# atoms-ufrj/atomsmm

Hardware: AMD Instinct MI355X
Metric: ns/day on 100k-atom TIP3P RESPA box; near-nonbonded HBM GB/s vs 8 TB/s peak (higher is better)
Workload: dtype f64

## Files before the change

### atomsmm_amd/csrc/cluster.h

```cpp
#pragma once
#include "amm_ctx.h"

struct ClusterList {
    int nc = 0;
    const int *d_first = nullptr;
    const int *d_rest = nullptr;
    int nrest = 0;
    bool built = false;
    CellGrid grid;
    int capc = 0;
    int parts = 1;
    int *d_slice_cells = nullptr;
    int split_parts = 0;
    double rext = 0;
    double rlist_build = 0, rnear_build = 0, skin = 0;
    int *d_cell_count = nullptr, *d_cell_start = nullptr, *d_cell_members = nullptr;
    int *d_cperm = nullptr;
    int *d_aperm = nullptr;
    float4 *d_pos4f = nullptr;
    double *d_xref = nullptr;
    int c_begin = 0, c_end = 0;
    int cap = 0;
    int lpa = 8;
    int *d_nl = nullptr, *d_nnb = nullptr, *d_nnb_near = nullptr;
    int *d_flags = nullptr;
    unsigned long long *d_counters = nullptr;
    unsigned long long *d_blockstats = nullptr;
    int *d_ticket = nullptr;
    long checked_epoch = -1, pre_epoch = -1;
    const double *checked_pos = nullptr, *pre_pos = nullptr;
    PairForce *sorted_for = nullptr;
    long sorted_epoch = -1;
    const double *sorted_pos = nullptr;
    int *d_spec_count[2] = {nullptr, nullptr};
    int *d_spec_ticket = nullptr;
    int spec_parity = 0;
    long assigned_epoch = -1;
    const double *assigned_pos = nullptr;
    double built_L[3] = {0, 0, 0};
// ... 14 lines not shown
```

### atomsmm_amd/csrc/cluster.hip

```cpp
#include <algorithm>
#include <cmath>
#include <cstdio>
#include <cstdlib>
#include <cstring>
#include <type_traits>
#include <vector>

#include "amm_ctx.h"
#include "bonded_terms.h"
#include "cluster.h"
#include "device_utils.h"
#include "pair_math.h"
#include "pair_tab.h"

#ifndef AMM_EXP_NOLJ
#define AMM_EXP_NOLJ 0
#endif

__device__ double amm_erfcx_table_dev_c[AMM_ERFCX_NI * AMM_ERFCX_NC];
static bool g_erfcx_uploaded_c[64] = {false};

void amm_cluster_classify(int n, const std::vector<int> &ptr, const std::vector<int> &idx, std::vector<int> &mol_first, std::vector<int> &rest) {
    mol_first.clear();
    rest.clear();
// ... 69 lines not shown

__device__ __forceinline__ double csorted_image(double x, double x0, double sh, double L, double invL) {
    return x + (sh - L * rint((x - x0) * invL));
}

__device__ __forceinline__ void cgather_one(int c, int i0, const double *__restrict__ pos, Box box, const double *__restrict__ q,
                                            const double *__restrict__ hsig, const double *__restrict__ seps2, double4 *posq_s, double2 *lj_s) {
    double sh[3];
#pragma unroll
    for (int k = 0; k < 3; ++k) sh[k] = cwrap1(pos[3 * i0 + k], box.L[k], box.invL[k]) - pos[3 * i0 + k];
#pragma unroll
    for (int a = 0; a < 3; ++a) {
        const int i = i0 + a;
        double4 p;
        p.x = csorted_image(pos[3 * i], pos[3 * i0], sh[0], box.L[0], box.invL[0]);
        p.y = csorted_image(pos[3 * i + 1], pos[3 * i0 + 1], sh[1], box.L[1], box.invL[1]);
        p.z = csorted_image(pos[3 * i + 2], pos[3 * i0 + 2], sh[2], box.L[2], box.invL[2]);
        p.w = q[i];
        posq_s[3 * c + a] = p;
        lj_s[3 * c + a] = make_double2(hsig[i], seps2[i]);
    }
}

__global__ void __launch_bounds__(256) k_csort_gather(int ncell, int nc, const int *__restrict__ start, const int *__restrict__ members,
                                                      int capc, int *cperm, int *aperm, const double *__restrict__ pos, Box box,
                                                      float4 *pos4f, const int *flags, int *wflags, int force, const double *__restrict__ q,
                                                      const double *__restrict__ hsig, const double *__restrict__ seps2, double4 *posq_s,
                                                      double2 *lj_s, float rext, const double *__restrict__ site_eps,
                                                      const int *__restrict__ first, CZeroRows Z, int copies_current, double *xref,
                                                      int c_begin, int c_end, int *slice_cells) {
    const int gid = blockIdx.x * blockDim.x + threadIdx.x;
    if (gid < Z.n) {
        const int i = Z.idx[gid];
        if (Z.f0) Z.f0[3 * i] = Z.f0[3 * i + 1] = Z.f0[3 * i + 2] = 0.0;
        if (Z.f1) Z.f1[3 * i] = Z.f1[3 * i + 1] = Z.f1[3 * i + 2] = 0.0;
    }
    if (!force && !flags[0]) {
        if (!copies_current && posq_s && gid < nc) cgather_one(gid, cfirst(first, cperm[gid]), pos, box, q, hsig, seps2, posq_s, lj_s);
        return;
    }
    const int wave = gid >> 6, lane = threadIdx.x & 63;
    if (wave >= ncell) return;
    const int b = start[wave];
    const int cnt = min(start[wave + 1] - b, capc);
    if (lane == 0 && c_begin < c_end) {
        if (b <= c_begin && c_begin < start[wave + 1]) slice_cells[0] = wave;
        if (b <= c_end - 1 && c_end - 1 < start[wave + 1]) slice_cells[1] = wave;
    }
    const int *mem = members + (size_t)wave * capc;
    for (int a0 = 0; a0 < cnt; a0 += 64) {
        const int a = a0 + lane;
        const int me = a < cnt ? mem[a] : 0x7fffffff;
        int rank = 0;
// ... 25 lines not shown
            const double z = csorted_image(pos[3 * i + 2], p0[2], sh[2], box.L[2], box.invL[2]);
            if (xref) {
                xref[3 * i] = pos[3 * i];
                xref[3 * i + 1] = pos[3 * i + 1];
                xref[3 * i + 2] = pos[3 * i + 2];
            }
            pf[t] = make_float4((float)x, (float)y, (float)z, 0.f);
            const float dx = pf[t].x - pf[0].x, dy = pf[t].y - pf[0].y, dz = pf[t].z - pf[0].z;
            ext2 = fmaxf(ext2, dx * dx + dy * dy + dz * dz);
            if (site_eps[i] != 0.0) sites |= 1 << t;
            if (posq_s) {
                posq_s[3 * sl + t] = make_double4(x, y, z, q[i]);
                lj_s[3 * sl + t] = make_double2(hsig[i], seps2[i]);
            }
        }
        const float ext = sqrtf(ext2) * 1.000001f + 1e-6f;
        if (!(ext <= rext)) wflags[7] = 1;
        pf[0].w = ext;
        pf[1].w = __int_as_float(sites);
        pos4f[3 * sl] = pf[0];
        pos4f[3 * sl + 1] = pf[1];
        pos4f[3 * sl + 2] = pf[2];
    }
}

struct CBoxF {
    float L[3], invL[3];
};

#ifndef CB_BATCH
#define CB_BATCH 5
#endif
#define CB_COARSE 256
#define CB_QCAP 256
__device__ __forceinline__ int cq_wrap(int i) { return i & (CB_QCAP - 1); }
typedef float v2f __attribute__((ext_vector_type(2)));

__device__ void cfinish_build_block(int *flags, unsigned long long *counters, const unsigned long long *blockstats, int nblocks, int count_only) {
    __shared__ unsigned long long sh_part[4][3];
    unsigned long long sum = 0, mx = 0, nr = 0;
    for (int b0 = threadIdx.x; b0 < nblocks; b0 += 8 * 256) {
        unsigned long long v[8][3];
#pragma unroll
        for (int j = 0; j < 8; ++j) {
            const int b = b0 + j * 256;
            const bool in = b < nblocks;
#pragma unroll
            for (int q = 0; q < 3; ++q) v[j][q] = in ? amm_ld_l2(&blockstats[3 * (in ? b : 0) + q]) : 0ull;
        }
#pragma unroll
        for (int j = 0; j < 8; ++j) {
            sum += v[j][0];
            mx = max(mx, v[j][1]);
            nr += v[j][2];
        }
    }
// ... 14 lines not shown
        counters[2] = sh_part[0][2] + sh_part[1][2] + sh_part[2][2] + sh_part[3][2];
        if (!count_only) {
            flags[0] = 0;
            flags[AMM_FLAG_FAR] = 0;
            counters[0] += 1;
        }
    }
}

#ifndef CB_WAVES
#define CB_WAVES 5
#endif
#define CB_OCC __attribute__((amdgpu_waves_per_eu(CB_WAVES)))
#ifdef AMM_CBS_TIMING
__device__ unsigned long long g_cbs_t[8];
#define CBS_STAMP(i) do { const unsigned long long now_ = wall_clock64(); if (w == 0 && lane == 0) atomicAdd(&g_cbs_t[i], now_ - t_last); t_last = now_; } while (0)
#else
#define CBS_STAMP(i) do { } while (0)
#endif
template <bool COUNT_ONLY, bool RINT, bool SLICE = false>
__global__ void __launch_bounds__(256) __attribute__((amdgpu_waves_per_eu(SLICE ? 3 : CB_WAVES))) k_cbuild(int c_begin, int c_end, int parts, const int *__restrict__ cell_start,
                                                const float4 *__restrict__ pos4f, CBoxF box, CellGrid g, float rlist, float rnear2, int cap,
                                                int *nl, int *nnb, int *nnb_near, int *flags, unsigned long long *blockstats,
                                                unsigned long long *counters, int *ticket, int force, const int *slice_cells) {
    if (!force && !flags[0]) return;
    __shared__ int s_rstart[4][128];
    __shared__ int s_rpref[4][128];
    __shared__ float s_rshift[4][3][128];
    __shared__ int s_q[4][CB_BATCH][CB_QCAP];
    __shared__ unsigned char s_coarse[4][CB_COARSE];
    const int lane = threadIdx.x & 63, w = threadIdx.x >> 6;
    const int wave = __builtin_amdgcn_readfirstlane((int)((blockIdx.x * blockDim.x + threadIdx.x) >> 6));
    const float FAR = 1.0e9f;
    const float rlist2 = rlist * rlist;
    unsigned long long wsum = 0, wnear = 0;
    int wmax = 0;
    const int first_cell = SLICE ? __builtin_amdgcn_readfirstlane(slice_cells[0]) : 0;
    const int nunits = SLICE ? (__builtin_amdgcn_readfirstlane(slice_cells[1]) - first_cell + 1) * parts : g.ncell * parts;
    int unit = wave;
#ifdef AMM_CBS_TIMING
    unsigned long long t_last = wall_clock64(), t_drain = 0, n_drain = 0;
#endif
    do {
    const int c = unit < nunits ? first_cell + unit / parts : g.ncell, part = unit % parts;
    int a_begin = 0, a_end = 0;
    if (c < g.ncell) {
        const int cb0 = __builtin_amdgcn_readfirstlane(cell_start[c]), cb1 = __builtin_amdgcn_readfirstlane(cell_start[c + 1]);
        const int per = (cb1 - cb0 + parts - 1) / parts;
        a_begin = max(cb0 + part * per, c_begin);
        a_end = min(min(cb0 + (part + 1) * per, cb1), c_end);
    }
    if (a_begin < a_end) {
        const int ncx = g.nc[0], ncy = g.nc[1], ncz = g.nc[2];
        const int cx = c % ncx, cy = (c / ncx) % ncy, cz = c / (ncx * ncy);
        const int nsx = g.nstencil[0], nsy = g.nstencil[1], ne = nsx * nsy * g.nstencil[2];
        int total;
        {
            int ecs[2] = {0, 0}, len[2] = {0, 0}, inc[2];
            float esx[2] = {0.f, 0.f}, esy[2] = {0.f, 0.f}, esz[2] = {0.f, 0.f};
#pragma unroll
            for (int hh = 0; hh < 2; ++hh) {
                const int e = lane + 64 * hh;
                if (e < ne) {
                    const int ox = e % nsx, oy = (e / nsx) % nsy, oz = e / (nsx * nsy);
                    int nz = ncz < 2 * g.h[2] + 1 ? oz : cz - g.h[2] + oz;
                    esz[hh] = nz < 0 ? -box.L[2] : (nz >= ncz ? box.L[2] : 0.f);
                    nz = nz < 0 ? nz + ncz : (nz >= ncz ? nz - ncz : nz);
                    int ny = ncy < 2 * g.h[1] + 1 ? oy : cy - g.h[1] + oy;
                    esy[hh] = ny < 0 ? -box.L[1] : (ny >= ncy ? box.L[1] : 0.f);
                    ny = ny < 0 ? ny + ncy : (ny >= ncy ? ny - ncy : ny);
                    int nx = ncx < 2 * g.h[0] + 1 ? ox : cx - g.h[0] + ox;
                    esx[hh] = nx < 0 ? -box.L[0] : (nx >= ncx ? box.L[0] : 0.f);
                    nx = nx < 0 ? nx + ncx : (nx >= ncx ? nx - ncx : nx);
                    const int cc = (nz * ncy + ny) * ncx + nx;
                    ecs[hh] = cell_start[cc];
                    len[hh] = cell_start[cc + 1] - ecs[hh];
                }
                inc[hh] = len[hh];
                for (int off = 1; off < 64; off <<= 1) {
                    const int v = __shfl_up(inc[hh], off);
                    if (lane >= off) inc[hh] += v;
                }
            }
            const int lower = __builtin_amdgcn_readlane(inc[0], 63);
            total = lower + __builtin_amdgcn_readlane(inc[1], 63);
#pragma unroll
            for (int hh = 0; hh < 2; ++hh) {
                s_rstart[w][lane + 64 * hh] = ecs[hh];
                s_rpref[w][lane + 64 * hh] = (hh ? lower : 0) + inc[hh] - len[hh];
                s_rshift[w][0][lane + 64 * hh] = esx[hh];
                s_rshift[w][1][lane + 64 * hh] = esy[hh];
                s_rshift[w][2][lane + 64 * hh] = esz[hh];
            }
            __builtin_amdgcn_fence(__ATOMIC_RELEASE, "wavefront");
            __builtin_amdgcn_wave_barrier();
            __builtin_amdgcn_fence(__ATOMIC_ACQUIRE, "wavefront");
        }
        int cshift = 3;
        while (((total + 127) >> cshift) > CB_COARSE) ++cshift;
#pragma unroll
        for (int q = 0; q < CB_COARSE / 64; ++q) {
            const int idx = (lane + 64 * q) << cshift;
            int r = 0;
#pragma unroll
            for (int step = 64; step > 0; step >>= 1)
                if (s_rpref[w][r + step] <= idx) r += step;
            s_coarse[w][lane + 64 * q] = (unsigned char)r;
        }
        __builtin_amdgcn_fence(__ATOMIC_RELEASE, "wavefront");
        __builtin_amdgcn_wave_barrier();
        __builtin_amdgcn_fence(__ATOMIC_ACQUIRE, "wavefront");
#ifdef AMM_CBS_TIMING
        if (SLICE && lane == 0) { atomicAdd(&g_cbs_t[7], 1ull); atomicAdd(&g_cbs_t[0], wall_clock64() - t_last); }
#endif
        for (int tb = a_begin; tb < a_end; tb += CB_BATCH) {
            const int nt = min(CB_BATCH, a_end - tb);
            float4 my = make_float4(0.f, 0.f, 0.f, 0.f);
            if (lane < 3 * nt) my = pos4f[3 * tb + lane];
            int row_cnt = 0;
            int q_head = 0, q_cnt = 0;
            auto rl = [&](float v, int l) { return __int_as_float(__builtin_amdgcn_readlane(__float_as_int(v), l)); };
            auto drain = [&](int t, int n) {
#ifdef AMM_CBS_TIMING
                const unsigned long long t_d0 = wall_clock64();
                n_drain++;
#endif
                const int head = __builtin_amdgcn_readlane(q_head, t);
                int slot[2];
                bool v[2];
                float4 A[2][3];
#pragma unroll
                for (int u = 0; u < 2; ++u) {
                    const bool v0 = lane + 64 * u < n;
                    slot[u] = v0 ? s_q[w][t][cq_wrap(head + lane + 64 * u)] : tb + t;
                    v[u] = v0 && slot[u] != tb + t;
                }
#pragma unroll
                for (int u = 0; u < 2; ++u)
#pragma unroll
                    for (int b = 0; b < 3; ++b) A[u][b] = pos4f[3 * slot[u] + b];
                const int sites[2] = {__float_as_int(A[0][1].w), __float_as_int(A[1][1].w)};
                float px[3], py[3], pz[3];
#pragma unroll
                for (int a = 0; a < 3; ++a) {
                    px[a] = rl(my.x, 3 * t + a);
                    py[a] = rl(my.y, 3 * t + a);
                    pz[a] = rl(my.z, 3 * t + a);
                }
                v2f ax[3], ay[3], az[3];
#pragma unroll
                for (int b = 0; b < 3; ++b) {
                    ax[b] = v2f{A[0][b].x, A[1][b].x};
                    ay[b] = v2f{A[0][b].y, A[1][b].y};
                    az[b] = v2f{A[0][b].z, A[1][b].z};
                }
                if (!RINT) {
                    const v2f sx = box.L[0] * __builtin_elementwise_rint((ax[0] - px[0]) * box.invL[0]);
                    const v2f sy = box.L[1] * __builtin_elementwise_rint((ay[0] - py[0]) * box.invL[1]);
                    const v2f sz = box.L[2] * __builtin_elementwise_rint((az[0] - pz[0]) * box.invL[2]);
#pragma unroll
                    for (int b = 0; b < 3; ++b) {
                        ax[b] -= sx;
                        ay[b] -= sy;
                        az[b] -= sz;
                    }
                }
                v2f m2 = v2f{3.0e38f, 3.0e38f};
#pragma unroll
                for (int a = 0; a < 3; ++a)
#pragma unroll
                    for (int b = 0; b < 3; ++b) {
                        v2f dx = px[a] - ax[b], dy = py[a] - ay[b], dz = pz[a] - az[b];
                        if (RINT) {
                            dx -= box.L[0] * __builtin_elementwise_rint(dx * box.invL[0]);
                            dy -= box.L[1] * __builtin_elementwise_rint(dy * box.invL[1]);
                            dz -= box.L[2] * __builtin_elementwise_rint(dz * box.invL[2]);
                        }
                        v2f r2 = dx * dx;
                        r2 = __builtin_elementwise_fma(dy, dy, r2);
                        r2 = __builtin_elementwise_fma(dz, dz, r2);
                        m2 = __builtin_elementwise_min(m2, r2);
                    }
#pragma unroll
                for (int u = 0; u < 2; ++u) {
                    const float m2u = u ? m2.y : m2.x;
                    const bool pass = v[u] && m2u < rlist2;
                    const unsigned long long m_pass = __builtin_amdgcn_ballot_w64(pass);
                    if (m_pass != 0ull) {
                        const bool is_near = pass && m2u < rnear2;
                        const unsigned long long m_near = __builtin_amdgcn_ballot_w64(is_near);
                        const int np_ = __popcll(m_pass), nn_ = __popcll(m_near);
                        const int c2 = __builtin_amdgcn_readlane(row_cnt, t);
                        const int cnt = c2 & 0xffff, cntf = (int)((unsigned)c2 >> 16);
                        if (!COUNT_ONLY) {
                            const int mp = __builtin_amdgcn_mbcnt_hi((unsigned)(m_pass >> 32), __builtin_amdgcn_mbcnt_lo((unsigned)m_pass, 0u));
                            const int mn = __builtin_amdgcn_mbcnt_hi((unsigned)(m_near >> 32), __builtin_amdgcn_mbcnt_lo((unsigned)m_near, 0u));
                            const int pos_near = cnt + mn, pos_far = (cap - 1 - cntf) - (mp - mn);
                            if (cnt + cntf + np_ <= cap) {
                                int *row_out = nl + (size_t)(tb + t - c_begin) * cap;
                                if (pass) row_out[is_near ? pos_near : pos_far] = slot[u] | (sites[u] << 29);
                            }
                        }
                        row_cnt = lane == t ? c2 + nn_ + ((np_ - nn_) << 16) : row_cnt;
                    }
                }
                q_head = lane == t ? cq_wrap(head + n) : q_head;
                q_cnt = lane == t ? q_cnt - n : q_cnt;
#ifdef AMM_CBS_TIMING
// ... 38 lines not shown
                        dx -= box.L[0] * __builtin_elementwise_rint(dx * box.invL[0]);
                        dy -= box.L[1] * __builtin_elementwise_rint(dy * box.invL[1]);
                        dz -= box.L[2] * __builtin_elementwise_rint(dz * box.invL[2]);
                    }
                    v2f r2 = dx * dx;
                    r2 = __builtin_elementwise_fma(dy, dy, r2);
                    r2 = __builtin_elementwise_fma(dz, dz, r2);
                    const v2f lim = plim + cw;
                    const v2f lim2 = lim * lim;
#pragma unroll
                    for (int u = 0; u < 2; ++u) {
                        const bool pass = (u ? r2.y < lim2.y : r2.x < lim2.x) && (!RINT || (u ? lim.y : lim.x) > 0.f);
                        const unsigned long long m = __builtin_amdgcn_ballot_w64(pass);
                        if (m == 0ull) continue;
                        const int at = qn + __builtin_amdgcn_mbcnt_hi((unsigned)(m >> 32), __builtin_amdgcn_mbcnt_lo((unsigned)m, 0u));
                        if (pass) s_q[w][t][cq_wrap(head + at)] = js[u];
                        qn += __popcll(m);
                    }
                    q_cnt = lane == t ? qn : q_cnt;
                    if (qn >= 128) {
                        __builtin_amdgcn_fence(__ATOMIC_RELEASE, "wavefront");
                        __builtin_amdgcn_wave_barrier();
                        __builtin_amdgcn_fence(__ATOMIC_ACQUIRE, "wavefront");
                        drain(t, 128);
                    }
                }
#pragma unroll
                for (int u = 0; u < 2; ++u) {
                    cand[u] = cand_n[u];
                    js[u] = js_n[u];
                }
            }
            __builtin_amdgcn_fence(__ATOMIC_RELEASE, "wavefront");
            __builtin_amdgcn_wave_barrier();
            __builtin_amdgcn_fence(__ATOMIC_ACQUIRE, "wavefront");
            for (int t = 0; t < nt; ++t) {
                const int n = __builtin_amdgcn_readlane(q_cnt, t);
                if (n > 0) drain(t, n);
            }
            __builtin_amdgcn_fence(__ATOMIC_RELEASE, "wavefront");
            __builtin_amdgcn_wave_barrier();
            if (lane < nt) {
                const int count = row_cnt & 0xffff, countf = (int)((unsigned)row_cnt >> 16);
                const int total_nb = count + countf;
                if (!COUNT_ONLY) {
                    const bool over = total_nb > cap;
                    nnb[tb + lane - c_begin] = over ? 0 : total_nb;
                    nnb_near[tb + lane - c_begin] = over ? 0 : count;
                    if (over) flags[1] = 1;
                }
                wsum += (unsigned long long)total_nb;
                wnear += (unsigned long long)count;
                wmax = max(wmax, total_nb);
            }
        }
    }
#ifdef AMM_CBS_TIMING
    if (SLICE && lane == 0 && a_begin < a_end) { atomicAdd(&g_cbs_t[1], wall_clock64() - t_last); atomicAdd(&g_cbs_t[2], t_drain); atomicAdd(&g_cbs_t[3], n_drain); }
#endif
    unit += (int)(gridDim.x * (blockDim.x >> 6));
    } while (SLICE && unit < nunits);
// ... 1367 lines not shown
        g.cw[k] = L / nc;
        g.inv_cw[k] = nc / L;
        g.ncell *= nc;
        if (!(rc + cl->skin + 2.0 * cl->rext < 0.5 * L * (1 - 1e-9))) cl->per_pair_image = true;
    }
    return 0;
}

static int cluster_chain(amm_ctx *ctx, PairForce *L, ClusterList *cl, const double *d_pos, int force, bool count_only, PairForce *gather_for,
                         CZeroRows Z = CZeroRows{0, nullptr, nullptr, nullptr}, int copies_current = 0, bool skip_assign = false) {
    hipStream_t st = ctx->stream;
    const int nc = cl->nc;
    if (!skip_assign)
        hipLaunchKernelGGL(k_cassign, dim3((nc + cl->nrest + 255) / 256), dim3(256), 0, st, nc, d_pos, ctx->box, cl->grid, cl->d_cell_count, cl->d_cell_start,
                           cl->d_cell_members, cl->capc, count_only ? (double *)nullptr : cl->d_xref, cl->d_flags, cl->d_ticket, force, cl->d_first,
                           cl->d_rest, cl->nrest);
    if (!cl->d_cell_members) return 0;
    PairForce *gf = gather_for;
    const long sort_threads = std::max(std::max((long)cl->grid.ncell * 64, gf ? (long)nc : 0L), (long)Z.n);
    hipLaunchKernelGGL(k_csort_gather, dim3((unsigned)((sort_threads + 255) / 256)), dim3(256), 0, st, cl->grid.ncell, nc, cl->d_cell_start,
                       cl->d_cell_members, cl->capc, cl->d_cperm, cl->d_aperm, d_pos, ctx->box, cl->d_pos4f, cl->d_flags, cl->d_flags, force,
                       gf ? gf->d_q : nullptr, gf ? gf->d_hsig : nullptr, gf ? gf->d_seps2 : nullptr, gf ? gf->d_posq_s : (double4 *)nullptr,
                       gf ? gf->d_lj_s : (double2 *)nullptr, (float)cl->rext, L->d_seps2, cl->d_first, Z, copies_current,
                       count_only ? (double *)nullptr : cl->d_xref, cl->c_begin, cl->c_end, cl->d_slice_cells);
    const bool slice = cl->c_end - cl->c_begin < cl->nc;
    const bool split = cl->split_parts > 0 && !count_only;
    const int ncell_grid = slice ? (int)std::min<long>(cl->grid.ncell, (5L * cl->grid.ncell) / (4L * std::max(1, ctx->world)) + 4) : cl->grid.ncell;
    const long threads = (long)ncell_grid * cl->parts * 64;
    dim3 grid(split ? (unsigned)(ncell_grid * cl->split_parts) : (unsigned)((threads + 255) / 256));
    CBoxF bf;
    for (int k = 0; k < 3; ++k) {
        bf.L[k] = (float)ctx->box.L[k];
        bf.invL[k] = (float)ctx->box.invL[k];
    }
    const float rl = (float)cl->rlist_build;
    const float rn2 = cl->rnear_build > 0 ? (float)(cl->rnear_build * cl->rnear_build) : 3.0e38f;
    const bool use_rint = cl->grid.nc[0] < 5 || cl->grid.nc[1] < 5 || cl->grid.nc[2] < 5;
#define AMM_LAUNCH_CBUILD(CO, RI)                                                                                                   \
    do {                                                                                                                            \
        if (slice)                                                                                                                  \
            hipLaunchKernelGGL((k_cbuild<CO, RI, true>), grid, dim3(256), 0, st, cl->c_begin, cl->c_end, cl->parts, cl->d_cell_start,    \
                               cl->d_pos4f, bf, cl->grid, rl, rn2, cl->cap, cl->d_nl, cl->d_nnb, cl->d_nnb_near, cl->d_flags,            \
                               cl->d_blockstats, cl->d_counters, cl->d_ticket + AMM_TICKET_INTS, force, cl->d_slice_cells);              \
        else                                                                                                                        \
            hipLaunchKernelGGL((k_cbuild<CO, RI, false>), grid, dim3(256), 0, st, cl->c_begin, cl->c_end, cl->parts, cl->d_cell_start,   \
                               cl->d_pos4f, bf, cl->grid, rl, rn2, cl->cap, cl->d_nl, cl->d_nnb, cl->d_nnb_near, cl->d_flags,            \
                               cl->d_blockstats, cl->d_counters, cl->d_ticket + AMM_TICKET_INTS, force, cl->d_slice_cells);              \
    } while (0)
#define AMM_LAUNCH_CBUILD_SPLIT(RI)                                                                                                  \
    hipLaunchKernelGGL((k_cbuild_split<RI>), grid, dim3(256), 0, st, cl->c_begin, cl->c_end, cl->split_parts, cl->d_cell_start,     \
                       cl->d_pos4f, bf, cl->grid, rl, rn2, cl->cap, cl->d_nl, cl->d_nnb, cl->d_nnb_near, cl->d_flags, cl->d_blockstats,  \
                       cl->d_counters, cl->d_ticket + AMM_TICKET_INTS, force, cl->d_slice_cells)
    if (count_only) {
        if (use_rint) AMM_LAUNCH_CBUILD(true, true);
        else AMM_LAUNCH_CBUILD(true, false);
    } else if (split) {
        if (use_rint) AMM_LAUNCH_CBUILD_SPLIT(true);
        else AMM_LAUNCH_CBUILD_SPLIT(false);
    } else {
        if (use_rint) AMM_LAUNCH_CBUILD(false, true);
        else AMM_LAUNCH_CBUILD(false, false);
    }
#undef AMM_LAUNCH_CBUILD
#undef AMM_LAUNCH_CBUILD_SPLIT
    AMM_HIP(hipGetLastError());
    return 0;
}

static double cluster_extent_host(amm_ctx *ctx, const double *d_pos, int n, int nc, const std::vector<int> &first) {
    std::vector<double> x(3 * (size_t)n);
// ... 46 lines not shown
    AMM_HIP(hipMalloc(&cl->d_pos4f, sizeof(float4) * 3 * (size_t)nc));
    AMM_HIP(hipMalloc(&cl->d_xref, sizeof(double) * 3 * (size_t)n));
    AMM_HIP(hipMalloc(&cl->d_nnb, sizeof(int) * ns));
    AMM_HIP(hipMalloc(&cl->d_nnb_near, sizeof(int) * ns));
    AMM_HIP(hipMalloc(&cl->d_flags, sizeof(int) * 16));
    AMM_HIP(hipMemset(cl->d_flags, 0, sizeof(int) * 16));
    AMM_HIP(hipMalloc(&cl->d_ticket, sizeof(int) * 4 * AMM_TICKET_INTS));
    AMM_HIP(hipMemset(cl->d_ticket, 0, sizeof(int) * 4 * AMM_TICKET_INTS));
    AMM_HIP(hipMalloc(&cl->d_counters, sizeof(unsigned long long) * 8));
    AMM_HIP(hipMemset(cl->d_counters, 0, sizeof(unsigned long long) * 8));
    AMM_HIP(hipMalloc(&cl->d_slice_cells, sizeof(int) * 2));
    AMM_HIP(hipMemset(cl->d_slice_cells, 0, sizeof(int) * 2));
    int lpa = 4;
    while (lpa < 64 && (long)(cl->c_end - cl->c_begin) * lpa < 64L * 2048) lpa <<= 1;
    if (ctx->opt_lpa > 0) lpa = ctx->opt_lpa;
    cl->lpa = lpa;
    int flags[8];
    cl->capc = 0;
    if (cluster_chain(ctx, L, cl, d_pos, 1, true, nullptr)) return 1;
    AMM_HIP(hipMemcpyAsync(flags, cl->d_flags, sizeof(flags), hipMemcpyDeviceToHost, ctx->stream));
    AMM_HIP(hipStreamSynchronize(ctx->stream));
    cl->capc = 2 * flags[6] + 16;
    AMM_HIP(hipMalloc(&cl->d_cell_members, sizeof(int) * (size_t)ncell * cl->capc));
    cl->parts = std::max(1, std::min(16, (int)std::ceil(1.5 * (double)nc / ncell / CB_BATCH)));
    if (ctx->world > 1) {
        const int active_cells = std::max(1, ncell / ctx->world);
        const int want = (4096 + active_cells - 1) / active_cells, most = std::max(1, (int)std::ceil((double)nc / ncell));
        cl->parts = std::max(cl->parts, std::min(want, std::min(most, 6)));
    }
    if (ctx->opt_parts > 0) cl->parts = std::max(1, std::min(16, ctx->opt_parts));
    cl->split_parts = 0;
    if (ctx->world > 1 && ctx->opt_build_split < 0) {
        const int active_cells = std::max(1, ncell / ctx->world);
        const int most = std::max(1, (int)std::ceil((double)nc / ncell / CBS_BATCH));
        cl->split_parts = std::max(1, std::min(std::min(16, most), (1024 + active_cells / 2) / active_cells));
    }
    if (ctx->opt_build_split == 0) cl->split_parts = 0;
    if (ctx->opt_build_split > 0) cl->split_parts = std::min(16, ctx->opt_build_split);
    {
        const long t1 = (long)ncell * cl->parts * 64;
        const size_t nblocks = std::max((size_t)((t1 + 255) / 256), (size_t)ncell * (size_t)cl->split_parts);
        AMM_HIP(hipMalloc(&cl->d_blockstats, sizeof(unsigned long long) * 3 * nblocks));
    }
    cl->cap = 0;
    {
        const int cb = cl->c_begin, ce = cl->c_end;
// ... 61 lines not shown
    }
    ClusterList *cl = L->cl;
    const EpiPlan *plan = ctx->epi_request;
    ctx->epi_request = nullptr;
    ctx->epi_done = false;
    const int copies_current = (cl->sorted_for == pf && cl->sorted_epoch == ctx->pos_epoch && cl->sorted_pos == d_pos && Z.n == 0) ? 1 : 0;
    if (copies_current) ctx->n_copies_current++;
    if (cl->checked_epoch == ctx->pos_epoch && cl->checked_pos == d_pos && !L->force_rebuild_c) {
    } else {
        if (!(cl->pre_epoch == ctx->pos_epoch && cl->pre_pos == d_pos))
            hipLaunchKernelGGL(k_ccheck_displacement, dim3((n + 255) / 256), dim3(256), 0, st, n, d_pos, cl->d_xref, 0.25 * cl->skin * cl->skin,
                               cl->d_flags);
        const int forced = L->force_rebuild_c ? 1 : 0;
        L->force_rebuild_c = false;
        const bool assigned = !forced && cl->assigned_epoch == ctx->pos_epoch && cl->assigned_pos == d_pos;
        if (cluster_chain(ctx, L, cl, d_pos, forced, false, pf, Z, copies_current, assigned)) return 1;
        gathered = true;
    }
    cl->checked_epoch = ctx->pos_epoch;
    cl->checked_pos = d_pos;
    if (!gathered && !copies_current)
        hipLaunchKernelGGL(k_csort_gather, dim3((std::max(cl->nc, Z.n) + 255) / 256), dim3(256), 0, st, cl->grid.ncell, cl->nc, cl->d_cell_start,
                           cl->d_cell_members, cl->capc, cl->d_cperm, cl->d_aperm, d_pos, ctx->box, cl->d_pos4f, cl->d_flags + 8, cl->d_flags, 0,
                           pf->d_q, pf->d_hsig, pf->d_seps2, pf->d_posq_s, pf->d_lj_s, (float)cl->rext, L->d_seps2, cl->d_first, Z, 0, (double *)nullptr, 0, 0, (int *)nullptr);
    cl->sorted_for = pf;
    cl->sorted_epoch = ctx->pos_epoch;
    cl->sorted_pos = d_pos;
    const int nrows = cl->c_end - cl->c_begin;
    const int per_c = (cl->nc + ctx->world - 1) / ctx->world, per = 3 * per_c, nf = guest ? 2 : 1;
    double *out = d_force, *gout = g_force;
    auto ss_bytes_of = [](const PairForce *p) { return (p->d_tab_ss && p->pc.tab.ss_first >= 0) ? (p->pc.tab.nint - p->pc.tab.ss_first) * AMM_TAB_STRIDE : 0; };
    auto plan_fits = [&]() {
        if (!(plan && plan->kind == 0 && ctx->opt_fuse_epilogue && !accumulate && !cl->d_first && cl->nrest == 0 && plan->bs && plan->bs->mol3_ok &&
              plan->bs->finalized && plan->bs->ncomp == cl->nc && plan->f0 && plan->npre <= AMM_MAX_PRE && ctx->d_x == d_pos && ctx->d_v &&
              plan->f0 != d_force && plan->f0 != g_force)) return false;
        if (guest && !(!g_accumulate && g_force != d_force && ctx->opt_fuse_rows && pf == L && cl->rnear_build > 0)) return false;
        return true;
    };
    bool state_mode = false;
    if (exchange && ctx->world > 1 && ctx->opt_state_exchange && plan_fits() && cl->nc - per_c * (ctx->world - 1) > 0) {
        bool kernel = ctx->opt_site_tab && ss_bytes_of(pf) > 0 && (!guest || ss_bytes_of(guest) > 0);
        const int lds = pf->pc.tab.nint * AMM_TAB_STRIDE + ss_bytes_of(pf) + (guest ? guest->pc.tab.nint * AMM_TAB_STRIDE + ss_bytes_of(guest) : 0);
        kernel = kernel && lds <= AMM_CPAIR_LDS_LIMIT;
        if (guest) kernel = kernel && guest->pc.family == AMM_NEAR_FSWITCH && (pf->pc.family == AMM_DAMPED || pf->pc.family == AMM_NONBONDED);
        state_mode = kernel;
    }
    if (state_mode) {
// ... 286 lines not shown
        const int back = A.cap - 1 + nfront;
        for (int k = sub; k < nn; k += 8) {
            const unsigned j = (unsigned)row[k < nfront ? k : back - k] & 0x1fffffffu;
            for (int t = 0; t < 3; ++t)
                for (int b = 0; b < 3; ++b) {
                    const double4 pi = A.posq[3 * cs + t], pj = A.posq[3 * j + b];
                    const double dx = amm_min_image(pi.x - pj.x, A.box.L[0], A.box.invL[0]);
                    const double dy = amm_min_image(pi.y - pj.y, A.box.L[1], A.box.invL[1]);
                    const double dz = amm_min_image(pi.z - pj.z, A.box.L[2], A.box.invL[2]);
                    cnt += (dx * dx + dy * dy + dz * dz < r2w) ? 1ull : 0ull;
                }
        }
    }
    for (int off = 32; off > 0; off >>= 1) cnt += __shfl_xor(cnt, off);
    if ((threadIdx.x & 63) == 0 && cnt) atomicAdd(out, cnt);
}

int amm_cluster_count_within_impl(amm_ctx *ctx, PairForce *pf, const double *d_pos, double r_within, long long *count) {
    PairForce *L = pf->host ? pf->host : pf;
    ClusterList *cl = L->cl;
    hipStream_t st = ctx->stream;
    hipLaunchKernelGGL(k_csort_gather, dim3((cl->nc + 255) / 256), dim3(256), 0, st, cl->grid.ncell, cl->nc, cl->d_cell_start, cl->d_cell_members,
                       cl->capc, cl->d_cperm, cl->d_aperm, d_pos, ctx->box, cl->d_pos4f, cl->d_flags + 8, cl->d_flags, 0, pf->d_q, pf->d_hsig,
                       pf->d_seps2, pf->d_posq_s, pf->d_lj_s, (float)cl->rext, L->d_seps2, cl->d_first, CZeroRows{0, nullptr, nullptr, nullptr}, 0, (double *)nullptr, 0, 0, (int *)nullptr);
    if (cl->sorted_for == pf) {
        cl->sorted_epoch = ctx->pos_epoch;
        cl->sorted_pos = d_pos;
    }
    CPairArgs A;
    std::memset(&A, 0, sizeof(A));
    A.c_begin = cl->c_begin;
    A.nrows = cl->c_end - cl->c_begin;
    A.cap = cl->cap;
    A.nl = cl->d_nl;
    A.nnb = (pf == L) ? cl->d_nnb : cl->d_nnb_near;
    A.nnb_total = nullptr;
    if (pf == L && cl->rnear_build > 0) {
        A.nnb = cl->d_nnb_near;
        A.nnb_total = cl->d_nnb;
    }
    A.posq = pf->d_posq_s;
    A.box = ctx->box;
    unsigned long long *d_cnt = cl->d_counters + 7;
    AMM_HIP(hipMemsetAsync(d_cnt, 0, sizeof(unsigned long long), st));
    if (A.nrows > 0)
        hipLaunchKernelGGL(k_ccount_within, dim3((unsigned)(((long)A.nrows * 8 + 255) / 256)), dim3(256), 0, st, A, r_within * r_within, d_cnt);
    unsigned long long h = 0;
// ... 42 lines not shown
    AMM_HIP(hipMemcpyAsync(h, d_out, sizeof(h), hipMemcpyDeviceToHost, st));
    AMM_HIP(hipStreamSynchronize(st));
    out[0] = (long long)h[0];
    out[1] = (long long)h[1];
    return 0;
}

int amm_cluster_free(ClusterList *cl) {
#ifdef AMM_CBS_TIMING
    {
        unsigned long long t[8];
        const bool got = hipMemcpyFromSymbol(t, HIP_SYMBOL(g_cbs_t), sizeof(t)) == hipSuccess && t[7];
        if (got && cl->split_parts == 0)
            fprintf(stderr, "k_cbuild<SLICE>: %llu busy wavefronts, mean: prologue %.2f us, whole %.2f us, in drains %.2f us (%.2f drains)\n", t[7], t[0] / 100.0 / t[7],
                    t[1] / 100.0 / t[7], t[2] / 100.0 / t[7], (double)t[3] / t[7]);
        if (got && cl->split_parts > 0)
            fprintf(stderr, "k_cbuild_split, first wavefront of %llu busy blocks, mean clocks (100 MHz): prologue %.2f | pass 1 %.2f wait %.2f | pass 2 %.2f wait %.2f | copy %.2f wait %.2f us\n",
                    t[7], t[0] / 100.0 / t[7], t[1] / 100.0 / t[7], t[2] / 100.0 / t[7], t[3] / 100.0 / t[7], t[4] / 100.0 / t[7], t[5] / 100.0 / t[7], t[6] / 100.0 / t[7]);
    }
#endif
    for (void *q : {(void *)cl->d_spec_count[0], (void *)cl->d_spec_count[1], (void *)cl->d_spec_ticket})
        if (q) (void)hipFree(q);
    if (cl->d_slice_cells) (void)hipFree(cl->d_slice_cells);
    void *ptrs[] = {cl->d_cell_count, cl->d_cell_start, cl->d_cell_members, cl->d_cperm, cl->d_aperm, cl->d_pos4f, cl->d_xref, cl->d_nl,
                    cl->d_nnb, cl->d_nnb_near, cl->d_flags, cl->d_counters, cl->d_blockstats, cl->d_ticket};
    for (void *p : ptrs)
        if (p) (void)hipFree(p);
    delete cl;
    return 0;
}
```

### atomsmm_amd/csrc/pair.hip

```cpp
#include <atomic>
#include <cmath>
#include <cstdio>
#include <cstdlib>
#include <cstring>

#include "amm_ctx.h"
#include "bonded_terms.h"
#include "cluster.h"
#include "device_utils.h"
#include "pair_args.h"
#include "pair_math.h"
#include "pair_tab.h"

int amm_pair_build_consts(const amm_pair_desc &d, PairConsts &pc) {
    pc.family = d.family;
    pc.flags = d.flags;
    pc.degree = d.degree < 1 ? 1 : d.degree;
    pc.cmode = (d.flags & AMM_COULOMB_EWALD) ? 1 : ((d.flags & AMM_COULOMB_RF) ? 2 : 0);
    pc.sign = d.sign;
    pc.rc = d.rc;
    pc.rc2 = d.rc * d.rc;
    pc.rc0 = d.rc0;
    pc.rs0 = d.rs0;
    pc.inv_dr0 = (d.rc0 > d.rs0) ? 1.0 / (d.rc0 - d.rs0) : 0.0;
// ... 1940 lines not shown
    A.s_end = L->s_end;
    A.lpa_shift = 3;
    A.cap = L->cap;
    A.nl = L->d_nl;
    A.nnb = L->d_nnb_near;
    A.nnb_total = (pf == L && L->rnear_build > 0) ? L->d_nnb : nullptr;
    A.posq_s = pf->d_posq_s;
    A.box = ctx->box;
    const int nslice = L->s_end - L->s_begin;
    unsigned long long *d_cnt = L->d_counters + 7;
    AMM_HIP(hipMemsetAsync(d_cnt, 0, sizeof(unsigned long long), st));
    if (nslice > 0)
        hipLaunchKernelGGL(k_count_within, dim3((unsigned)(((long)nslice * 8 + 255) / 256)), dim3(256), 0, st, A, r_within * r_within, nslice, d_cnt);
    unsigned long long h = 0;
    AMM_HIP(hipMemcpyAsync(&h, d_cnt, sizeof(h), hipMemcpyDeviceToHost, st));
    AMM_HIP(hipStreamSynchronize(st));
    *count = (long long)h;
    return 0;
}

extern "C" __attribute__((weak)) const char *amm_variant_tag(void);
const char *amm_kernel_revision_impl() {
#ifdef AMM_CLUSTER_TUNE
    return "r07-triploop-tune";
#else
    return amm_variant_tag ? "r07-triploop-tune" : "r07-triploop";
#endif
}

int amm_pair_build_table(PairForce *pf) {
    std::vector<double> coef;
    SiteTable ss;
    ss.want = pf->cluster_ok && pf->one_site_class && pf->site_one_charge && pf->site_q != 0.0 && pf->site_seps2 != 0.0;
    ss.sig = 2.0 * pf->site_hsig;
    ss.eps4 = pf->site_seps2 * pf->site_seps2;
    ss.QQ = pf->pc.Kc * pf->site_q * pf->site_q;
    pf->tab_error = amm_build_coulomb_table(pf->pc, coef, &ss);
    pf->ss_built_for[0] = pf->site_hsig;
    pf->ss_built_for[1] = pf->site_seps2;
    pf->ss_built_for[2] = ss.want ? pf->site_q : 0.0;
    if (pf->d_tab) {
        (void)hipFree(pf->d_tab);
        pf->d_tab = nullptr;
    }
    if (pf->d_tab_ss) {
        (void)hipFree(pf->d_tab_ss);
        pf->d_tab_ss = nullptr;
    }
    pf->ss_error = ss.error;
// ... 99 lines not shown
```

Before: 1155.

## Precompute per-cell stencil tables in sort kernel and add single-vector drain path

Each cell's neighbour-stencil data (run starts, prefix sums, coarse search index and periodic-shift codes) is now computed once, in k_csort_gather, and stored in a per-cell CBuildTab record. k_cbuild then loads that record in 16-byte pieces instead of having every part-wave recompute it. The first batch's positions are also fetched earlier so the load overlaps with the table setup. A single-lane-slot drain variant handles queue tails of 64 or fewer entries, avoiding wasted packed work. The cost is an extra per-cell buffer and more work in the sort kernel. The other k_csort_gather call sites pass a null table pointer, which is only safe while those calls never reach the table-building path.

After: 1168, median of 6. +1.1%, better.

```diff
diff --git a/atomsmm_amd/csrc/cluster.h b/atomsmm_amd/csrc/cluster.h
--- a/atomsmm_amd/csrc/cluster.h
+++ b/atomsmm_amd/csrc/cluster.h
@@ -1,5 +1,7 @@
 #pragma once
 #include "amm_ctx.h"
+
+struct CBuildTab;
 
 struct ClusterList {
     int nc = 0;
@@ -15,6 +17,7 @@
     double rext = 0;
     double rlist_build = 0, rnear_build = 0, skin = 0;
     int *d_cell_count = nullptr, *d_cell_start = nullptr, *d_cell_members = nullptr;
+    CBuildTab *d_build_tabs = nullptr;
     int *d_cperm = nullptr;
     int *d_aperm = nullptr;
     float4 *d_pos4f = nullptr;
diff --git a/atomsmm_amd/csrc/cluster.hip b/atomsmm_amd/csrc/cluster.hip
--- a/atomsmm_amd/csrc/cluster.hip
+++ b/atomsmm_amd/csrc/cluster.hip
@@ -115,13 +115,89 @@
     }
 }
 
+#define CB_COARSE 256
+#ifndef CB_HALF_DRAIN
+#define CB_HALF_DRAIN 1
+#endif
+struct alignas(16) CBuildTab {
+    int rstart[128];
+    int rpref[128];
+    unsigned char coarse[CB_COARSE];
+    unsigned short code[64];
+    int total, cshift, pad[2];
+};
+static_assert(sizeof(CBuildTab) == 1424 && offsetof(CBuildTab, rpref) == 512 && offsetof(CBuildTab, coarse) == 1024, "k_cbuild loads the record in 16-byte pieces");
+
+__device__ __forceinline__ float cshift_of(int code2, float L) { return code2 == 0 ? -L : (code2 == 2 ? L : 0.f); }
+
+__device__ __forceinline__ void cbuild_tables(int c, int lane, const CellGrid &g, const int *__restrict__ cell_start, int *s_pref, CBuildTab *out) {
+    const int ncx = g.nc[0], ncy = g.nc[1], ncz = g.nc[2];
+    const int cx = c % ncx, cy = (c / ncx) % ncy, cz = c / (ncx * ncy);
+    const int nsx = g.nstencil[0], nsy = g.nstencil[1], ne = nsx * nsy * g.nstencil[2];
+    int ecs[2] = {0, 0}, len[2] = {0, 0}, inc[2], code[2] = {0x15, 0x15};
+#pragma unroll
+    for (int hh = 0; hh < 2; ++hh) {
+        const int e = lane + 64 * hh;
+        if (e < ne) {
+            const int ox = e % nsx, oy = (e / nsx) % nsy, oz = e / (nsx * nsy);
+            int nz = ncz < 2 * g.h[2] + 1 ? oz : cz - g.h[2] + oz;
+            const int kz = nz < 0 ? 0 : (nz >= ncz ? 2 : 1);
+            nz = nz < 0 ? nz + ncz : (nz >= ncz ? nz - ncz : nz);
+            int ny = ncy < 2 * g.h[1] + 1 ? oy : cy - g.h[1] + oy;
+            const int ky = ny < 0 ? 0 : (ny >= ncy ? 2 : 1);
+            ny = ny < 0 ? ny + ncy : (ny >= ncy ? ny - ncy : ny);
+            int nx = ncx < 2 * g.h[0] + 1 ? ox : cx - g.h[0] + ox;
+            const int kx = nx < 0 ? 0 : (nx >= ncx ? 2 : 1);
+            nx = nx < 0 ? nx + ncx : (nx >= ncx ? nx - ncx : nx);
+            const int cc = (nz * ncy + ny) * ncx + nx;
+            ecs[hh] = cell_start[cc];
+            len[hh] = cell_start[cc + 1] - ecs[hh];
+            code[hh] = kx | (ky << 2) | (kz << 4);
+        }
+        inc[hh] = len[hh];
+        for (int off = 1; off < 64; off <<= 1) {
+            const int v = __shfl_up(inc[hh], off);
+            if (lane >= off) inc[hh] += v;
+        }
+    }
+    const int lower = __builtin_amdgcn_readlane(inc[0], 63);
+    const int total = lower + __builtin_amdgcn_readlane(inc[1], 63);
+#pragma unroll
+    for (int hh = 0; hh < 2; ++hh) {
+        const int pref = (hh ? lower : 0) + inc[hh] - len[hh];
+        out->rstart[lane + 64 * hh] = ecs[hh];
+        out->rpref[lane + 64 * hh] = pref;
+        s_pref[lane + 64 * hh] = pref;
+    }
+    out->code[lane] = (unsigned short)(code[0] | (code[1] << 8));
+    __builtin_amdgcn_fence(__ATOMIC_RELEASE, "wavefront");
+    __builtin_amdgcn_wave_barrier();
+    __builtin_amdgcn_fence(__ATOMIC_ACQUIRE, "wavefront");
+    int cshift = 3;
+    while (((total + 127) >> cshift) > CB_COARSE) ++cshift;
+#pragma unroll
+    for (int q = 0; q < CB_COARSE / 64; ++q) {
+        const int idx = (lane + 64 * q) << cshift;
+        int r = 0;
+#pragma unroll
+        for (int step = 64; step > 0; step >>= 1)
+            if (s_pref[r + step] <= idx) r += step;
+        out->coarse[lane + 64 * q] = (unsigned char)r;
+    }
+    if (lane == 0) {
+        out->total = total;
+        out->cshift = cshift;
+    }
+}
+
 __global__ void __launch_bounds__(256) k_csort_gather(int ncell, int nc, const int *__restrict__ start, const int *__restrict__ members,
                                                       int capc, int *cperm, int *aperm, const double *__restrict__ pos, Box box,
                                                       float4 *pos4f, const int *flags, int *wflags, int force, const double *__restrict__ q,
                                                       const double *__restrict__ hsig, const double *__restrict__ seps2, double4 *posq_s,
                                                       double2 *lj_s, float rext, const double *__restrict__ site_eps,
                                                       const int *__restrict__ first, CZeroRows Z, int copies_current, double *xref,
-                                                      int c_begin, int c_end, int *slice_cells) {
+                                                      int c_begin, int c_end, int *slice_cells, CellGrid g, CBuildTab *tabs) {
+    __shared__ int s_pref[4][128];
     const int gid = blockIdx.x * blockDim.x + threadIdx.x;
     if (gid < Z.n) {
         const int i = Z.idx[gid];
@@ -193,6 +269,7 @@
         pos4f[3 * sl + 1] = pf[1];
         pos4f[3 * sl + 2] = pf[2];
     }
+    cbuild_tables(__builtin_amdgcn_readfirstlane(wave), lane, g, start, s_pref[threadIdx.x >> 6], tabs + wave);
 }
 
 struct CBoxF {
@@ -202,7 +279,6 @@
 #ifndef CB_BATCH
 #define CB_BATCH 5
 #endif
-#define CB_COARSE 256
 #define CB_QCAP 256
 __device__ __forceinline__ int cq_wrap(int i) { return i & (CB_QCAP - 1); }
 typedef float v2f __attribute__((ext_vector_type(2)));
@@ -263,13 +339,14 @@
 __global__ void __launch_bounds__(256) __attribute__((amdgpu_waves_per_eu(SLICE ? 3 : CB_WAVES))) k_cbuild(int c_begin, int c_end, int parts, const int *__restrict__ cell_start,
                                                 const float4 *__restrict__ pos4f, CBoxF box, CellGrid g, float rlist, float rnear2, int cap,
                                                 int *nl, int *nnb, int *nnb_near, int *flags, unsigned long long *blockstats,
-                                                unsigned long long *counters, int *ticket, int force, const int *slice_cells) {
+                                                unsigned long long *counters, int *ticket, int force, const int *slice_cells,
+                                                const CBuildTab *__restrict__ tabs) {
     if (!force && !flags[0]) return;
-    __shared__ int s_rstart[4][128];
-    __shared__ int s_rpref[4][128];
+    __shared__ __attribute__((aligned(16))) int s_rstart[4][128];
+    __shared__ __attribute__((aligned(16))) int s_rpref[4][128];
     __shared__ float s_rshift[4][3][128];
     __shared__ int s_q[4][CB_BATCH][CB_QCAP];
-    __shared__ unsigned char s_coarse[4][CB_COARSE];
+    __shared__ __attribute__((aligned(16))) unsigned char s_coarse[4][CB_COARSE];
     const int lane = threadIdx.x & 63, w = threadIdx.x >> 6;
     const int wave = __builtin_amdgcn_readfirstlane((int)((blockIdx.x * blockDim.x + threadIdx.x) >> 6));
     const float FAR = 1.0e9f;
@@ -292,62 +369,20 @@
         a_end = min(min(cb0 + (part + 1) * per, cb1), c_end);
     }
     if (a_begin < a_end) {
-        const int ncx = g.nc[0], ncy = g.nc[1], ncz = g.nc[2];
-        const int cx = c % ncx, cy = (c / ncx) % ncy, cz = c / (ncx * ncy);
-        const int nsx = g.nstencil[0], nsy = g.nstencil[1], ne = nsx * nsy * g.nstencil[2];
-        int total;
-        {
-            int ecs[2] = {0, 0}, len[2] = {0, 0}, inc[2];
-            float esx[2] = {0.f, 0.f}, esy[2] = {0.f, 0.f}, esz[2] = {0.f, 0.f};
-#pragma unroll
-            for (int hh = 0; hh < 2; ++hh) {
-                const int e = lane + 64 * hh;
-                if (e < ne) {
-                    const int ox = e % nsx, oy = (e / nsx) % nsy, oz = e / (nsx * nsy);
-                    int nz = ncz < 2 * g.h[2] + 1 ? oz : cz - g.h[2] + oz;
-                    esz[hh] = nz < 0 ? -box.L[2] : (nz >= ncz ? box.L[2] : 0.f);
-                    nz = nz < 0 ? nz + ncz : (nz >= ncz ? nz - ncz : nz);
-                    int ny = ncy < 2 * g.h[1] + 1 ? oy : cy - g.h[1] + oy;
-                    esy[hh] = ny < 0 ? -box.L[1] : (ny >= ncy ? box.L[1] : 0.f);
-                    ny = ny < 0 ? ny + ncy : (ny >= ncy ? ny - ncy : ny);
-                    int nx = ncx < 2 * g.h[0] + 1 ? ox : cx - g.h[0] + ox;
-                    esx[hh] = nx < 0 ? -box.L[0] : (nx >= ncx ? box.L[0] : 0.f);
-                    nx = nx < 0 ? nx + ncx : (nx >= ncx ? nx - ncx : nx);
-                    const int cc = (nz * ncy + ny) * ncx + nx;
-                    ecs[hh] = cell_start[cc];
-                    len[hh] = cell_start[cc + 1] - ecs[hh];
-                }
-                inc[hh] = len[hh];
-                for (int off = 1; off < 64; off <<= 1) {
-                    const int v = __shfl_up(inc[hh], off);
-                    if (lane >= off) inc[hh] += v;
-                }
-            }
-            const int lower = __builtin_amdgcn_readlane(inc[0], 63);
-            total = lower + __builtin_amdgcn_readlane(inc[1], 63);
-#pragma unroll
-            for (int hh = 0; hh < 2; ++hh) {
-                s_rstart[w][lane + 64 * hh] = ecs[hh];
-                s_rpref[w][lane + 64 * hh] = (hh ? lower : 0) + inc[hh] - len[hh];
-                s_rshift[w][0][lane + 64 * hh] = esx[hh];
-                s_rshift[w][1][lane + 64 * hh] = esy[hh];
-                s_rshift[w][2][lane + 64 * hh] = esz[hh];
-            }
-            __builtin_amdgcn_fence(__ATOMIC_RELEASE, "wavefront");
-            __builtin_amdgcn_wave_barrier();
-            __builtin_amdgcn_fence(__ATOMIC_ACQUIRE, "wavefront");
-        }
-        int cshift = 3;
-        while (((total + 127) >> cshift) > CB_COARSE) ++cshift;
-#pragma unroll
-        for (int q = 0; q < CB_COARSE / 64; ++q) {
-            const int idx = (lane + 64 * q) << cshift;
-            int r = 0;
-#pragma unroll
-            for (int step = 64; step > 0; step >>= 1)
-                if (s_rpref[w][r + step] <= idx) r += step;
-            s_coarse[w][lane + 64 * q] = (unsigned char)r;
-        }
+        const CBuildTab *__restrict__ tab = tabs + c;
+        const int total = __builtin_amdgcn_readfirstlane(tab->total), cshift = __builtin_amdgcn_readfirstlane(tab->cshift);
+        const int4 tab_rp = reinterpret_cast<const int4 *>(tab->rstart)[lane];
+        const int tab_co = reinterpret_cast<const int *>(tab->coarse)[lane];
+        const int tab_code = tab->code[lane];
+        const int nt0 = min(CB_BATCH, a_end - a_begin);
+        float4 my = pos4f[3 * a_begin + min(lane, 3 * nt0 - 1)];
+        if (lane >= 3 * nt0) my = make_float4(0.f, 0.f, 0.f, 0.f);
+        *reinterpret_cast<int4 *>(lane < 32 ? &s_rstart[w][4 * lane] : &s_rpref[w][4 * (lane - 32)]) = tab_rp;
+        reinterpret_cast<int *>(s_coarse[w])[lane] = tab_co;
+#pragma unroll
+        for (int hh = 0; hh < 2; ++hh)
+#pragma unroll
+            for (int k = 0; k < 3; ++k) s_rshift[w][k][lane + 64 * hh] = cshift_of((tab_code >> (8 * hh + 2 * k)) & 3, box.L[k]);
         __builtin_amdgcn_fence(__ATOMIC_RELEASE, "wavefront");
         __builtin_amdgcn_wave_barrier();
         __builtin_amdgcn_fence(__ATOMIC_ACQUIRE, "wavefront");
@@ -356,31 +391,39 @@
 #endif
         for (int tb = a_begin; tb < a_end; tb += CB_BATCH) {
             const int nt = min(CB_BATCH, a_end - tb);
-            float4 my = make_float4(0.f, 0.f, 0.f, 0.f);
-            if (lane < 3 * nt) my = pos4f[3 * tb + lane];
+            if (tb > a_begin) {
+                my = make_float4(0.f, 0.f, 0.f, 0.f);
+                if (lane < 3 * nt) my = pos4f[3 * tb + lane];
+            }
             int row_cnt = 0;
             int q_head = 0, q_cnt = 0;
             auto rl = [&](float v, int l) { return __int_as_float(__builtin_amdgcn_readlane(__float_as_int(v), l)); };
-            auto drain = [&](int t, int n) {
+            auto drain = [&](int t, int n, auto nu_) {
+                constexpr int NU = decltype(nu_)::value;
+                using V = typename std::conditional<NU == 2, v2f, float>::type;
+                auto pk = [](const float (&x)[NU]) -> V { if constexpr (NU == 2) return v2f{x[0], x[1]}; else return x[0]; };
+                auto half = [](V x, int u) -> float { if constexpr (NU == 2) return u ? x.y : x.x; else return x; };
 #ifdef AMM_CBS_TIMING
                 const unsigned long long t_d0 = wall_clock64();
                 n_drain++;
 #endif
                 const int head = __builtin_amdgcn_readlane(q_head, t);
-                int slot[2];
-                bool v[2];
-                float4 A[2][3];
-#pragma unroll
-                for (int u = 0; u < 2; ++u) {
+                int slot[NU];
+                bool v[NU];
+                float4 A[NU][3];
+#pragma unroll
+                for (int u = 0; u < NU; ++u) {
                     const bool v0 = lane + 64 * u < n;
                     slot[u] = v0 ? s_q[w][t][cq_wrap(head + lane + 64 * u)] : tb + t;
                     v[u] = v0 && slot[u] != tb + t;
                 }
 #pragma unroll
-                for (int u = 0; u < 2; ++u)
+                for (int u = 0; u < NU; ++u)
 #pragma unroll
                     for (int b = 0; b < 3; ++b) A[u][b] = pos4f[3 * slot[u] + b];
-                const int sites[2] = {__float_as_int(A[0][1].w), __float_as_int(A[1][1].w)};
+                int sites[NU];
+#pragma unroll
+                for (int u = 0; u < NU; ++u) sites[u] = __float_as_int(A[u][1].w);
                 float px[3], py[3], pz[3];
 #pragma unroll
                 for (int a = 0; a < 3; ++a) {
@@ -388,17 +431,24 @@
                     py[a] = rl(my.y, 3 * t + a);
                     pz[a] = rl(my.z, 3 * t + a);
                 }
-                v2f ax[3], ay[3], az[3];
+                V ax[3], ay[3], az[3];
 #pragma unroll
                 for (int b = 0; b < 3; ++b) {
-                    ax[b] = v2f{A[0][b].x, A[1][b].x};
-                    ay[b] = v2f{A[0][b].y, A[1][b].y};
-                    az[b] = v2f{A[0][b].z, A[1][b].z};
+                    float hx[NU], hy[NU], hz[NU];
+#pragma unroll
+                    for (int u = 0; u < NU; ++u) {
+                        hx[u] = A[u][b].x;
+                        hy[u] = A[u][b].y;
+                        hz[u] = A[u][b].z;
+                    }
+                    ax[b] = pk(hx);
+                    ay[b] = pk(hy);
+                    az[b] = pk(hz);
                 }
                 if (!RINT) {
-                    const v2f sx = box.L[0] * __builtin_elementwise_rint((ax[0] - px[0]) * box.invL[0]);
-                    const v2f sy = box.L[1] * __builtin_elementwise_rint((ay[0] - py[0]) * box.invL[1]);
-                    const v2f sz = box.L[2] * __builtin_elementwise_rint((az[0] - pz[0]) * box.invL[2]);
+                    const V sx = box.L[0] * __builtin_elementwise_rint((ax[0] - px[0]) * box.invL[0]);
+                    const V sy = box.L[1] * __builtin_elementwise_rint((ay[0] - py[0]) * box.invL[1]);
+                    const V sz = box.L[2] * __builtin_elementwise_rint((az[0] - pz[0]) * box.invL[2]);
 #pragma unroll
                     for (int b = 0; b < 3; ++b) {
                         ax[b] -= sx;
@@ -406,25 +456,27 @@
                         az[b] -= sz;
                     }
                 }
-                v2f m2 = v2f{3.0e38f, 3.0e38f};
+                V m2;
+                if constexpr (NU == 2) m2 = v2f{3.0e38f, 3.0e38f};
+                else m2 = 3.0e38f;
 #pragma unroll
                 for (int a = 0; a < 3; ++a)
 #pragma unroll
                     for (int b = 0; b < 3; ++b) {
-                        v2f dx = px[a] - ax[b], dy = py[a] - ay[b], dz = pz[a] - az[b];
+                        V dx = px[a] - ax[b], dy = py[a] - ay[b], dz = pz[a] - az[b];
                         if (RINT) {
                             dx -= box.L[0] * __builtin_elementwise_rint(dx * box.invL[0]);
                             dy -= box.L[1] * __builtin_elementwise_rint(dy * box.invL[1]);
                             dz -= box.L[2] * __builtin_elementwise_rint(dz * box.invL[2]);
                         }
-                        v2f r2 = dx * dx;
+                        V r2 = dx * dx;
                         r2 = __builtin_elementwise_fma(dy, dy, r2);
                         r2 = __builtin_elementwise_fma(dz, dz, r2);
                         m2 = __builtin_elementwise_min(m2, r2);
                     }
 #pragma unroll
-                for (int u = 0; u < 2; ++u) {
-                    const float m2u = u ? m2.y : m2.x;
+                for (int u = 0; u < NU; ++u) {
+                    const float m2u = half(m2, u);
                     const bool pass = v[u] && m2u < rlist2;
                     const unsigned long long m_pass = __builtin_amdgcn_ballot_w64(pass);
                     if (m_pass != 0ull) {
@@ -509,7 +561,7 @@
                         __builtin_amdgcn_fence(__ATOMIC_RELEASE, "wavefront");
                         __builtin_amdgcn_wave_barrier();
                         __builtin_amdgcn_fence(__ATOMIC_ACQUIRE, "wavefront");
-                        drain(t, 128);
+                        drain(t, 128, std::integral_constant<int, 2>());
                     }
                 }
 #pragma unroll
@@ -523,7 +575,12 @@
             __builtin_amdgcn_fence(__ATOMIC_ACQUIRE, "wavefront");
             for (int t = 0; t < nt; ++t) {
                 const int n = __builtin_amdgcn_readlane(q_cnt, t);
-                if (n > 0) drain(t, n);
+#if CB_HALF_DRAIN
+                if (n > 64) drain(t, n, std::integral_constant<int, 2>());
+                else if (n > 0) drain(t, n, std::integral_constant<int, 1>());
+#else
+                if (n > 0) drain(t, n, std::integral_constant<int, 2>());
+#endif
             }
             __builtin_amdgcn_fence(__ATOMIC_RELEASE, "wavefront");
             __builtin_amdgcn_wave_barrier();
@@ -1937,7 +1994,7 @@
                        cl->d_cell_members, cl->capc, cl->d_cperm, cl->d_aperm, d_pos, ctx->box, cl->d_pos4f, cl->d_flags, cl->d_flags, force,
                        gf ? gf->d_q : nullptr, gf ? gf->d_hsig : nullptr, gf ? gf->d_seps2 : nullptr, gf ? gf->d_posq_s : (double4 *)nullptr,
                        gf ? gf->d_lj_s : (double2 *)nullptr, (float)cl->rext, L->d_seps2, cl->d_first, Z, copies_current,
-                       count_only ? (double *)nullptr : cl->d_xref, cl->c_begin, cl->c_end, cl->d_slice_cells);
+                       count_only ? (double *)nullptr : cl->d_xref, cl->c_begin, cl->c_end, cl->d_slice_cells, cl->grid, cl->d_build_tabs);
     const bool slice = cl->c_end - cl->c_begin < cl->nc;
     const bool split = cl->split_parts > 0 && !count_only;
     const int ncell_grid = slice ? (int)std::min<long>(cl->grid.ncell, (5L * cl->grid.ncell) / (4L * std::max(1, ctx->world)) + 4) : cl->grid.ncell;
@@ -1956,11 +2013,13 @@
         if (slice)                                                                                                                  \
             hipLaunchKernelGGL((k_cbuild<CO, RI, true>), grid, dim3(256), 0, st, cl->c_begin, cl->c_end, cl->parts, cl->d_cell_start,    \
                                cl->d_pos4f, bf, cl->grid, rl, rn2, cl->cap, cl->d_nl, cl->d_nnb, cl->d_nnb_near, cl->d_flags,            \
-                               cl->d_blockstats, cl->d_counters, cl->d_ticket + AMM_TICKET_INTS, force, cl->d_slice_cells);              \
+                               cl->d_blockstats, cl->d_counters, cl->d_ticket + AMM_TICKET_INTS, force, cl->d_slice_cells,              \
+                               cl->d_build_tabs);                                                                                        \
         else                                                                                                                        \
             hipLaunchKernelGGL((k_cbuild<CO, RI, false>), grid, dim3(256), 0, st, cl->c_begin, cl->c_end, cl->parts, cl->d_cell_start,   \
                                cl->d_pos4f, bf, cl->grid, rl, rn2, cl->cap, cl->d_nl, cl->d_nnb, cl->d_nnb_near, cl->d_flags,            \
-                               cl->d_blockstats, cl->d_counters, cl->d_ticket + AMM_TICKET_INTS, force, cl->d_slice_cells);              \
+                               cl->d_blockstats, cl->d_counters, cl->d_ticket + AMM_TICKET_INTS, force, cl->d_slice_cells,              \
+                               cl->d_build_tabs);                                                                                        \
     } while (0)
 #define AMM_LAUNCH_CBUILD_SPLIT(RI)                                                                                                  \
     hipLaunchKernelGGL((k_cbuild_split<RI>), grid, dim3(256), 0, st, cl->c_begin, cl->c_end, cl->split_parts, cl->d_cell_start,     \
@@ -2053,6 +2112,7 @@
     AMM_HIP(hipStreamSynchronize(ctx->stream));
     cl->capc = 2 * flags[6] + 16;
     AMM_HIP(hipMalloc(&cl->d_cell_members, sizeof(int) * (size_t)ncell * cl->capc));
+    AMM_HIP(hipMalloc(&cl->d_build_tabs, sizeof(CBuildTab) * (size_t)ncell));
     cl->parts = std::max(1, std::min(16, (int)std::ceil(1.5 * (double)nc / ncell / CB_BATCH)));
     if (ctx->world > 1) {
         const int active_cells = std::max(1, ncell / ctx->world);
@@ -2160,7 +2220,7 @@
     if (!gathered && !copies_current)
         hipLaunchKernelGGL(k_csort_gather, dim3((std::max(cl->nc, Z.n) + 255) / 256), dim3(256), 0, st, cl->grid.ncell, cl->nc, cl->d_cell_start,
                            cl->d_cell_members, cl->capc, cl->d_cperm, cl->d_aperm, d_pos, ctx->box, cl->d_pos4f, cl->d_flags + 8, cl->d_flags, 0,
-                           pf->d_q, pf->d_hsig, pf->d_seps2, pf->d_posq_s, pf->d_lj_s, (float)cl->rext, L->d_seps2, cl->d_first, Z, 0, (double *)nullptr, 0, 0, (int *)nullptr);
+                           pf->d_q, pf->d_hsig, pf->d_seps2, pf->d_posq_s, pf->d_lj_s, (float)cl->rext, L->d_seps2, cl->d_first, Z, 0, (double *)nullptr, 0, 0, (int *)nullptr, cl->grid, (CBuildTab *)nullptr);
     cl->sorted_for = pf;
     cl->sorted_epoch = ctx->pos_epoch;
     cl->sorted_pos = d_pos;
@@ -2493,7 +2553,7 @@
     hipStream_t st = ctx->stream;
     hipLaunchKernelGGL(k_csort_gather, dim3((cl->nc + 255) / 256), dim3(256), 0, st, cl->grid.ncell, cl->nc, cl->d_cell_start, cl->d_cell_members,
                        cl->capc, cl->d_cperm, cl->d_aperm, d_pos, ctx->box, cl->d_pos4f, cl->d_flags + 8, cl->d_flags, 0, pf->d_q, pf->d_hsig,
-                       pf->d_seps2, pf->d_posq_s, pf->d_lj_s, (float)cl->rext, L->d_seps2, cl->d_first, CZeroRows{0, nullptr, nullptr, nullptr}, 0, (double *)nullptr, 0, 0, (int *)nullptr);
+                       pf->d_seps2, pf->d_posq_s, pf->d_lj_s, (float)cl->rext, L->d_seps2, cl->d_first, CZeroRows{0, nullptr, nullptr, nullptr}, 0, (double *)nullptr, 0, 0, (int *)nullptr, cl->grid, (CBuildTab *)nullptr);
     if (cl->sorted_for == pf) {
         cl->sorted_epoch = ctx->pos_epoch;
         cl->sorted_pos = d_pos;
@@ -2582,6 +2642,7 @@
     for (void *q : {(void *)cl->d_spec_count[0], (void *)cl->d_spec_count[1], (void *)cl->d_spec_ticket})
         if (q) (void)hipFree(q);
     if (cl->d_slice_cells) (void)hipFree(cl->d_slice_cells);
+    if (cl->d_build_tabs) (void)hipFree(cl->d_build_tabs);
     void *ptrs[] = {cl->d_cell_count, cl->d_cell_start, cl->d_cell_members, cl->d_cperm, cl->d_aperm, cl->d_pos4f, cl->d_xref, cl->d_nl,
                     cl->d_nnb, cl->d_nnb_near, cl->d_flags, cl->d_counters, cl->d_blockstats, cl->d_ticket};
     for (void *p : ptrs)
diff --git a/atomsmm_amd/csrc/pair.hip b/atomsmm_amd/csrc/pair.hip
--- a/atomsmm_amd/csrc/pair.hip
+++ b/atomsmm_amd/csrc/pair.hip
@@ -1986,9 +1986,9 @@
 extern "C" __attribute__((weak)) const char *amm_variant_tag(void);
 const char *amm_kernel_revision_impl() {
 #ifdef AMM_CLUSTER_TUNE
-    return "r07-triploop-tune";
+    return "r08-buildtabs-tune";
 #else
-    return amm_variant_tag ? "r07-triploop-tune" : "r07-triploop";
+    return amm_variant_tag ? "r08-buildtabs-tune" : "r08-buildtabs";
 #endif
 }
 
```
